# jarek1992/raytracer_project

Hardware: AMD Instinct MI355X
Metric: Msamples/sec (rays·bounces) (higher is better)
Workload: dtype f64

## Files before the change

raytracer_project_amd/csrc/zr_build.h:

```cpp
#pragma once
#include <hip/hip_runtime_api.h>
#include <stdint.h>

#include <vector>

#include "zr_device_types.h"

namespace zr {

struct BuildSceneIn {
    const double* spheres = nullptr; const uint32_t* sphere_mat = nullptr;
    const double* tri_v = nullptr; const double* tri_n = nullptr; const uint32_t* tri_mat = nullptr;
    const double* cubes = nullptr; const uint32_t* cube_mat = nullptr;
    const zr_medium* media = nullptr; const zr_xform_op* ops = nullptr;
    const double* group_box = nullptr;
};

struct BuildParams {
    float ct = 1.0f;
    float ck[8] = {1, 1.5f, 1, 3, 3, 1.5f, 16, 1};
    int max_leaf = 4;
    int leaf_cap[8] = {0, 0, 1, 1, 1, 1, 1, 0};
    float open_ratio = 1.25f;
    int radius = 16;
    int top_clusters = 16384;
};

struct BuildPrimOut {
    double* spheres = nullptr; uint32_t* sphere_mat = nullptr;
    double* tri_v = nullptr; double* tri_s = nullptr;
    double* cubes = nullptr; uint32_t* cube_mat = nullptr;
    double* pcubes = nullptr; uint32_t* pcube_mat = nullptr;
    DInstance* insts = nullptr; uint32_t* inst_group = nullptr;
    uint32_t base[8] = {0, 0, 0, 0, 0, 0, 0, 0};
    uint32_t* src[8] = {};
};

struct BuiltTree {
    NodePair* pairs = nullptr; uint32_t n_pairs = 0;
    NodeQ* quads = nullptr; uint32_t n_quads = 0;
    NodeF root{};
    double box[6] = {0, 0, 0, 0, 0, 0};
    uint32_t depth = 0;
    uint32_t quad_depth = 0;
    uint32_t demand = 0;
    bool quant_ok = true;
    uint32_t cnt[8] = {0, 0, 0, 0, 0, 0, 0, 0};
    std::vector<uint32_t> compound;
    double ms[8] = {0, 0, 0, 0, 0, 0, 0, 0};
    uint32_t ploc_iterations = 0;
    bool want_boxes = false;
    std::vector<float> dbg_boxes;
};

class DeviceBuilder {
public:
    explicit DeviceBuilder(hipStream_t stream) : st_(stream) {}
    ~DeviceBuilder();
    DeviceBuilder(const DeviceBuilder&) = delete;
    DeviceBuilder& operator=(const DeviceBuilder&) = delete;
    static size_t scratch_bytes(uint32_t n);
    hipError_t reserve(size_t bytes);
    hipError_t build(const BuildSceneIn& in, const zr_object* d_objects, const uint8_t* d_code, uint32_t first_triangle, uint32_t n,
                     const BuildParams& prm, bool root_in_array, const BuildPrimOut& out, const uint32_t* d_run_demand,
                     uint32_t depth_limit, bool stats, BuiltTree& t);
    hipError_t relocate(const BuiltTree& t, NodePair* pairs_dst, uint32_t pair_off, NodeQ* quads_dst, uint32_t quad_off);
    hipError_t patch_instances(DInstance* insts, const uint32_t* inst_group, uint32_t n, const uint32_t* d_run_root, const uint32_t* d_run_qroot);
    const char* error() const { return err_; }
    bool wants_host() const { return use_host_; }
    void* alloc_keep(size_t bytes);
private:
    hipStream_t st_;
    unsigned char* arena_ = nullptr; size_t arena_bytes_ = 0;
// ... 7 lines not shown
```

raytracer_project_amd/csrc/zr_build.hip:

```cpp
#include <cstring>
#include <hip/hip_runtime.h>
#include <rocprim/device/device_radix_sort.hpp>
#include <rocprim/device/device_scan.hpp>
#include <rocprim/iterator/counting_iterator.hpp>
#include <rocprim/iterator/transform_iterator.hpp>

#include <algorithm>
#include <chrono>
#include <cstdio>
#include <vector>

#include "zr_build.h"
#include "zr_bvh.h"

namespace zr {
namespace {

constexpr uint32_t NONE = 0xFFFFFFFFu;
constexpr int MAX_R = 32;
constexpr uint32_t M_KIND = 7u, M_UNIFORM = 8u, M_LEAF = 16u;

struct PBox { float lo[3]; uint32_t kind; float hi[3]; uint32_t pad; };
struct Cl { float lo[3]; uint32_t node; float hi[3]; uint32_t pad; };
struct BNode { float lo[3]; uint32_t left; float hi[3]; uint32_t right; };
static_assert(sizeof(PBox) == 32 && sizeof(Cl) == 32 && sizeof(BNode) == 32, "32-byte records: two 16-byte accesses");

struct Params {
    float ct; float ck[8]; int max_leaf; int cap[8]; float open_ratio; int radius;
};

__device__ __forceinline__ float f_down(double x) { return nextafterf(__double2float_rd(x), -__builtin_huge_valf()); }
__device__ __forceinline__ float f_up(double x) { return nextafterf(__double2float_ru(x), __builtin_huge_valf()); }
__device__ __forceinline__ float half_area(const float* lo, const float* hi) {
    const float dx = hi[0] - lo[0], dy = hi[1] - lo[1], dz = hi[2] - lo[2];
    return dx * dy + dy * dz + dz * dx;
}

struct DBox { double lo[3], hi[3]; };

__device__ DBox prim_box(const BuildSceneIn& in, uint32_t type, uint32_t idx);
__device__ DBox apply_op_box(const zr_xform_op& op, const DBox& b) {
    DBox o;
    if (op.kind == ZR_OP_TRANSLATE) { for (int k = 0; k < 3; k++) { o.lo[k] = b.lo[k] + op.a[k]; o.hi[k] = b.hi[k] + op.a[k]; } return o; }
    if (op.kind == ZR_OP_SCALE) {
        for (int k = 0; k < 3; k++) { const double a0 = b.lo[k] * op.a[k], a1 = b.hi[k] * op.a[k]; o.lo[k] = fmin(a0, a1); o.hi[k] = fmax(a0, a1); }
        return o;
    }
    if (op.kind == ZR_OP_MATERIAL) return b;
    const double sn = op.a[0], co = op.a[1];
    const int ia = op.kind == ZR_OP_ROTATE_X ? 1 : 0, ib = op.kind == ZR_OP_ROTATE_Z ? 1 : 2, ic = 3 - ia - ib;
    const double a0 = ia == 0 ? b.lo[0] : b.lo[1], a1 = ia == 0 ? b.hi[0] : b.hi[1];
// ... 367 lines not shown
        for (int k = 0; k < nk; k++) { lo[k] = bn[kids[k]].lo[ax]; hi[k] = bn[kids[k]].hi[ax]; }
        if (!quant_axis(lo, hi, nk, nq.origin[ax], nq.scale[ax], ql[ax], qh[ax])) return false;
        for (int k = 0; k < nk; k++) { nq.q[ax] |= ql[ax][k] << (8 * k); nq.q[3 + ax] |= qh[ax][k] << (8 * k); }
    }
    worst = 1;
    for (int k = 0; k < nk; k++) {
        double d[3];
        for (int ax = 0; ax < 3; ax++) d[ax] = plane_val(nq.origin[ax], nq.scale[ax], (int)qh[ax][k]) - plane_val(nq.origin[ax], nq.scale[ax], (int)ql[ax][k]);
        const double aq = d[0] * d[1] + d[1] * d[2] + d[2] * d[0];
        const BNode b = bn[kids[k]];
        const double at = (double)half_area(b.lo, b.hi);
        const float rr = at > 0 ? (float)(aq / at) : (aq > 0 ? 3.0e38f : 1.0f);
        if (!(rr <= worst)) worst = rr;
    }
    return true;
}

struct PlanOut {
    uint32_t counter;
    uint32_t quant_fail;
    uint32_t quad_depth;
    uint32_t kept_closed;
    uint32_t root_demand;
    uint32_t pad_[3];
    NodeF root;
};

__device__ __forceinline__ uint32_t leaf_ref(const uint32_t* __restrict__ nmeta, const uint32_t* __restrict__ ncount, const uint32_t* __restrict__ leaf_pos, uint32_t node) {
    return ZR_REF_LEAF | ((nmeta[node] & M_KIND) << 28) | ((ncount[node] - 1u) << 24) | leaf_pos[node];
}

__global__ __launch_bounds__(256) void k_plan(const BNode* __restrict__ bn, const uint32_t* __restrict__ nmeta, const uint32_t* __restrict__ ncount,
                                              const uint32_t* __restrict__ leaf_pos, uint32_t node_lo, uint32_t node_hi, uint32_t root, int root_in_array, float open_ratio,
                                              const zr_object* __restrict__ objs, const uint32_t* __restrict__ run_demand,
                                              uint32_t* __restrict__ qroot, uint32_t* __restrict__ qlevel, uint32_t* __restrict__ qinst, NodeQ* __restrict__ quads,
                                              PlanOut* __restrict__ po) {
    const uint32_t id = node_lo + blockIdx.x * 256 + threadIdx.x;
    if (id >= node_hi) return;
    const bool is_root = id == root;
    const bool fp32_root = is_root && !root_in_array;
    const uint32_t me = qroot[id];
    if (!fp32_root && me == NONE) return;
    uint32_t kids[4]; int nk = 0;
    NodeQ nq;
    for (int ax = 0; ax < 3; ax++) { nq.origin[ax] = 0; nq.scale[ax] = 1; }
    for (int k = 0; k < 6; k++) nq.q[k] = 0;
    float worst = 1;
    if (nmeta[id] & M_LEAF) {
        kids[nk++] = id;
        if (!fp32_root && !quantise(bn, kids, nk, nq, worst)) atomicExch(&po->quant_fail, 1u);
    } else {
        const BNode b = bn[id];
        kids[0] = b.left; kids[1] = b.right; nk = 2;
        if (!fp32_root && !quantise(bn, kids, nk, nq, worst)) atomicExch(&po->quant_fail, 1u);
        while (nk < 4) {
            int best = -1; float ba = -1;
            for (int k = 0; k < nk; k++) {
                if (nmeta[kids[k]] & M_LEAF) continue;
                const BNode c = bn[kids[k]];
                const float ar = half_area(c.lo, c.hi);
                if (ar > ba) { ba = ar; best = k; }
            }
            if (best < 0) break;
            uint32_t trial[4];
            for (int k = 0; k < nk; k++) trial[k] = kids[k];
            const BNode ob = bn[kids[best]];
            trial[best] = ob.left; trial[nk] = ob.right;
            if (!fp32_root) {
                NodeQ tq = nq; float w = 1;
                if (!quantise(bn, trial, nk + 1, tq, w)) { atomicExch(&po->quant_fail, 1u); break; }
                if (w > open_ratio && w > worst) { atomicAdd(&po->kept_closed, 1u); break; }
                nq = tq; worst = w;
            }
            for (int k = 0; k <= nk; k++) kids[k] = trial[k];
            nk++;
        }
    }
    int n_inner = 0;
    for (int k = 0; k < nk; k++) if (!(nmeta[kids[k]] & M_LEAF)) n_inner++;
    uint32_t next = n_inner ? atomicAdd(&po->counter, (uint32_t)n_inner) : 0u;
    const uint32_t my_level = fp32_root ? 0u : qlevel[me];
    uint32_t refs[4] = {ZR_REF_EMPTY, ZR_REF_EMPTY, ZR_REF_EMPTY, ZR_REF_EMPTY};
    uint32_t inst_demand = 0;
    for (int k = 0; k < nk; k++) {
        const uint32_t c = kids[k];
        if (nmeta[c] & M_LEAF) {
            refs[k] = leaf_ref(nmeta, ncount, leaf_pos, c);
            if ((nmeta[c] & M_KIND) == ZR_KIND_INSTANCE && run_demand && objs) {
                uint32_t q = c;
                while (bn[q].right != NONE) q = bn[q].left;
                const uint32_t g = objs[bn[q].left].index;
                const uint32_t d = 1u + run_demand[g];
                if (d > inst_demand) inst_demand = d;
            }
        } else { refs[k] = next; qroot[c] = next; qlevel[next] = my_level + 1u; next++; }
    }
    if (n_inner) atomicMax(&po->quad_depth, my_level + 1u);
    if (fp32_root) {
        NodeF rf;
// ... 212 lines not shown
}
__global__ __launch_bounds__(256) void k_fill_u32(uint32_t* __restrict__ a, size_t n, uint32_t v) {
    const size_t i = (size_t)blockIdx.x * 256 + threadIdx.x;
    if (i < n) a[i] = v;
}

inline dim3 grid_for(size_t n) { return dim3((unsigned)((n + 255) / 256)); }
double now_s() { return std::chrono::duration<double>(std::chrono::steady_clock::now().time_since_epoch()).count(); }

}

DeviceBuilder::~DeviceBuilder() {
    if (arena_) (void)hipFree(arena_);
    for (void* p : keep_) (void)hipFree(p);
}
void* DeviceBuilder::alloc_keep(size_t bytes) {
    void* p = nullptr;
    if (hipMalloc(&p, bytes < 64 ? 64 : bytes) != hipSuccess) { (void)hipGetLastError(); return nullptr; }
    keep_.push_back(p);
    return p;
}
size_t DeviceBuilder::scratch_bytes(uint32_t n) {
    const size_t N = 2 * (size_t)n + 2;
    return (size_t)n * (32 + 16 + 8 + 64 + 4 + 1 + 4 + 1 + 4 + 4 + 4 + 4 + 4 + 4 + 8) + N * (32 + 4 + 4 + 4 + 4 + 4 + 4) + (size_t)n * 24 + (64u << 20);
}
hipError_t DeviceBuilder::reserve(size_t bytes) {
    if (bytes <= arena_bytes_) return hipSuccess;
    if (arena_) { (void)hipStreamSynchronize(st_); (void)hipFree(arena_); arena_ = nullptr; arena_bytes_ = 0; }
    hipError_t e = hipMalloc((void**)&arena_, bytes);
    if (e != hipSuccess) { (void)hipGetLastError(); err_ = "out of device memory for the build's scratch"; return e; }
    arena_bytes_ = bytes;
    return hipSuccess;
}

hipError_t DeviceBuilder::build(const BuildSceneIn& in, const zr_object* d_objects, const uint8_t* d_code, uint32_t first_triangle, uint32_t n,
                                const BuildParams& bp, bool root_in_array, const BuildPrimOut& out, const uint32_t* d_run_demand, uint32_t depth_limit,
                                bool stats, BuiltTree& t) {
    hipError_t e;
    err_ = ""; use_host_ = false;
    if (n == 0) { err_ = "empty tree"; use_host_ = true; return hipErrorInvalidValue; }
    Params prm;
    prm.ct = bp.ct; prm.max_leaf = bp.max_leaf < 1 ? 1 : (bp.max_leaf > 16 ? 16 : bp.max_leaf); prm.open_ratio = bp.open_ratio;
    prm.radius = bp.radius < 1 ? 1 : (bp.radius > MAX_R ? MAX_R : bp.radius);
    for (int k = 0; k < 8; k++) { prm.ck[k] = bp.ck[k]; prm.cap[k] = bp.leaf_cap[k]; }
    const size_t N = 2 * (size_t)n;
    const uint32_t nb_max = (n + 255) / 256;
    PBox* pbox; uint64_t *keys_a, *keys_b; uint32_t *vals_a, *vals_b; Cl *cl_a, *cl_b; BNode* bn;
    uint32_t *parent, *ncount, *nmeta, *leaf_pos, *qroot, *nn, *blk_keep, *blk_new, *keep_off, *new_off, *dfs_obj, *rank, *scanned, *qlevel, *qinst, *qdem, *compound, *state;
    float* ncost; uint8_t *act, *dfs_kind; PlanOut* po; void* tmp; size_t tmp_bytes = 0;
    uint32_t *qinst_plan, *qmap, *qscan; NodeQ* quads_plan;
    auto layout = [&](unsigned char* base) -> size_t {
        unsigned char* at = base;
        auto take = [&](size_t bytes) { void* p = at; at += (bytes + 255) / 256 * 256; return p; };
        pbox = (PBox*)take((size_t)n * sizeof(PBox));
        keys_a = (uint64_t*)take((size_t)n * 8); keys_b = (uint64_t*)take((size_t)n * 8);
        vals_a = (uint32_t*)take((size_t)n * 4); vals_b = (uint32_t*)take((size_t)n * 4);
        cl_a = (Cl*)take((size_t)n * sizeof(Cl)); cl_b = (Cl*)take((size_t)n * sizeof(Cl));
        bn = (BNode*)take(N * sizeof(BNode));
        parent = (uint32_t*)take(N * 4); ncount = (uint32_t*)take(N * 4); nmeta = (uint32_t*)take(N * 4);
        ncost = (float*)take(N * 4);
        leaf_pos = (uint32_t*)take(N * 4); qroot = (uint32_t*)take(N * 4);
        nn = (uint32_t*)take((size_t)n * 4); act = (uint8_t*)take(n);
        blk_keep = (uint32_t*)take((size_t)nb_max * 4); blk_new = (uint32_t*)take((size_t)nb_max * 4);
        keep_off = (uint32_t*)take((size_t)nb_max * 4); new_off = (uint32_t*)take((size_t)nb_max * 4);
        dfs_obj = (uint32_t*)take((size_t)n * 4); dfs_kind = (uint8_t*)take(n);
        rank = (uint32_t*)take((size_t)n * 4); scanned = (uint32_t*)take((size_t)n * 4);
        qlevel = (uint32_t*)take((size_t)n * 4); qinst = (uint32_t*)take((size_t)n * 4); qdem = (uint32_t*)take((size_t)n * 4);
        qinst_plan = (uint32_t*)take((size_t)n * 4); qmap = (uint32_t*)take((size_t)n * 4); qscan = (uint32_t*)take(N * 4);
        quads_plan = (NodeQ*)take((size_t)n * sizeof(NodeQ));
        compound = (uint32_t*)take((size_t)n * 8);
        state = (uint32_t*)take(256);
        po = (PlanOut*)take(sizeof(PlanOut));
        if (tmp_bytes == 0) {
            size_t a = 0, b = 0, c = 0;
            (void)rocprim::radix_sort_pairs(nullptr, a, keys_a, keys_b, vals_a, vals_b, (size_t)n, 0, 63, st_);
            (void)rocprim::exclusive_scan(nullptr, b, rocprim::make_transform_iterator(dfs_kind, IsKind{0}), scanned, 0u, (size_t)n, rocprim::plus<uint32_t>(), st_);
            (void)rocprim::exclusive_scan(nullptr, c, rocprim::make_transform_iterator(rocprim::make_counting_iterator<uint32_t>(0u), InnerFlag{nmeta, 0}), scanned, 0u,
                                          (size_t)n, rocprim::plus<uint32_t>(), st_);
            size_t d = 0;
            (void)rocprim::exclusive_scan(nullptr, d, rocprim::make_transform_iterator(rocprim::make_counting_iterator<uint32_t>(0u), QRootFlag{qroot, 0}), qscan, 0u, N,
                                          rocprim::plus<uint32_t>(), st_);
            if (d > c) c = d;
            tmp_bytes = (a > b ? (a > c ? a : c) : (b > c ? b : c)) + 4096;
        }
        tmp = take(tmp_bytes);
        return (size_t)(at - base);
    };
    const size_t need = layout(nullptr);
    if ((e = reserve(need)) != hipSuccess) return e;
    (void)layout(arena_);
    double t0 = now_s();
    auto lap = [&](int k) { if (stats) { (void)hipStreamSynchronize(st_); const double t1 = now_s(); t.ms[k] += (t1 - t0) * 1e3; t0 = t1; } };
// ... 118 lines not shown
    const uint32_t quad_cap = n;
    NodeQ* quads = (NodeQ*)alloc_keep((size_t)quad_cap * sizeof(NodeQ));
    NodePair* pairs = (NodePair*)alloc_keep((size_t)n * sizeof(NodePair));
    if (!quads || !pairs) { err_ = "out of device memory for the tree's records"; return hipErrorOutOfMemory; }
    hipLaunchKernelGGL(k_fill_u32, grid_for(N), dim3(256), 0, st_, qroot, N, NONE);
    PlanOut h_po_in; std::memset(&h_po_in, 0, sizeof h_po_in);
    h_po_in.counter = root_in_array ? 1u : 0u;
    if ((e = hipMemcpyAsync(po, &h_po_in, sizeof h_po_in, hipMemcpyHostToDevice, st_)) != hipSuccess) return e;
    if ((e = hipMemsetAsync(qinst_plan, 0, (size_t)n * 4, st_)) != hipSuccess) return e;
    if ((e = hipMemsetAsync(qinst, 0, (size_t)n * 4, st_)) != hipSuccess) return e;
    if ((e = hipMemsetAsync(qdem, 0, (size_t)n * 4, st_)) != hipSuccess) return e;
    auto renumber = [&]() -> hipError_t {
        auto flags = rocprim::make_transform_iterator(rocprim::make_counting_iterator<uint32_t>(0u), QRootFlag{qroot, root});
        hipError_t er = rocprim::exclusive_scan(tmp, tmp_bytes, flags, qscan, 0u, (size_t)n_nodes, rocprim::plus<uint32_t>(), st_);
        if (er != hipSuccess) { err_ = "scan failed"; return er; }
        hipLaunchKernelGGL(k_qmap, grid_for(n_nodes), dim3(256), 0, st_, qroot, qscan, n_nodes, qmap);
        hipLaunchKernelGGL(k_qpermute, grid_for(quad_cap), dim3(256), 0, st_, quads_plan, quads, qinst_plan, qinst, qmap, quad_cap, po);
        return hipSuccess;
    };
    if (root_in_array) {
        if ((e = hipMemsetAsync(qroot + root, 0, 4, st_)) != hipSuccess) return e;
        if ((e = hipMemsetAsync(qlevel, 0, 4, st_)) != hipSuccess) return e;
    }
    if (n == 1) {
        hipLaunchKernelGGL(k_plan, dim3(1), dim3(256), 0, st_, bn, nmeta, ncount, leaf_pos, root, root + 1, root, root_in_array ? 1 : 0, prm.open_ratio, d_objects, d_run_demand,
                           qroot, qlevel, qinst_plan, quads_plan, po);
        if ((e = renumber()) != hipSuccess) return e;
        hipLaunchKernelGGL(k_demand, dim3(1), dim3(256), 0, st_, qroot, root, root + 1, root, root_in_array ? 1 : 0, quads, qinst, qdem, po);
    } else {
        for (size_t b = batch_start.size() - 1; b-- > 0;) {
            const uint32_t lo = batch_start[b], hi = batch_start[b + 1];
            hipLaunchKernelGGL(k_plan, grid_for(hi - lo), dim3(256), 0, st_, bn, nmeta, ncount, leaf_pos, lo, hi, root, root_in_array ? 1 : 0, prm.open_ratio, d_objects,
                               d_run_demand, qroot, qlevel, qinst_plan, quads_plan, po);
        }
        if ((e = renumber()) != hipSuccess) return e;
        for (size_t b = 0; b + 1 < batch_start.size(); b++) {
            const uint32_t lo = batch_start[b], hi = batch_start[b + 1];
            hipLaunchKernelGGL(k_demand, grid_for(hi - lo), dim3(256), 0, st_, qroot, lo, hi, root, root_in_array ? 1 : 0, quads, qinst, qdem, po);
        }
    }
    lap(4);
    uint32_t n_pairs = 1;
    if (n >= 2) {
        uint32_t h_root_meta = 0;
        if ((e = hipMemcpyAsync(&h_root_meta, nmeta + root, 4, hipMemcpyDeviceToHost, st_)) != hipSuccess) return e;
        if ((e = hipStreamSynchronize(st_)) != hipSuccess) return e;
        if (h_root_meta & M_LEAF) hipLaunchKernelGGL(k_pair_leaf_root, dim3(1), dim3(1), 0, st_, bn, nmeta, ncount, leaf_pos, root, pairs);
        else {
            auto flags = rocprim::make_transform_iterator(rocprim::make_counting_iterator<uint32_t>(0u), InnerFlag{nmeta, root});
            uint32_t* prank = scanned;
            if ((e = rocprim::exclusive_scan(tmp, tmp_bytes, flags, prank, 0u, (size_t)(n - 1), rocprim::plus<uint32_t>(), st_)) != hipSuccess) { err_ = "scan failed"; return e; }
            hipLaunchKernelGGL(k_pairs, grid_for(n - 1), dim3(256), 0, st_, bn, nmeta, ncount, leaf_pos, prank, n, pairs);
            uint32_t last = 0, last_meta = 0;
            if ((e = hipMemcpyAsync(&last, prank + (n - 2), 4, hipMemcpyDeviceToHost, st_)) != hipSuccess) return e;
            if ((e = hipMemcpyAsync(&last_meta, nmeta + n, 4, hipMemcpyDeviceToHost, st_)) != hipSuccess) return e;
            if ((e = hipStreamSynchronize(st_)) != hipSuccess) return e;
            n_pairs = last + ((last_meta & M_LEAF) ? 0u : 1u);
        }
    } else hipLaunchKernelGGL(k_pair_leaf_root, dim3(1), dim3(1), 0, st_, bn, nmeta, ncount, leaf_pos, root, pairs);
    lap(5);
    if ((e = hipMemsetAsync(state + 20, 0, 4, st_)) != hipSuccess) return e;
    hipLaunchKernelGGL(k_emit, grid_for(n), dim3(256), 0, st_, in, d_objects, d_code, first_triangle, n, dfs_obj, dfs_kind, rank, out, compound, state + 20);
    uint32_t n_compound = 0;
    BNode h_root;
    PlanOut h_po;
    if ((e = hipMemcpyAsync(&h_po, po, sizeof h_po, hipMemcpyDeviceToHost, st_)) != hipSuccess) return e;
    if ((e = hipMemcpyAsync(&n_compound, state + 20, 4, hipMemcpyDeviceToHost, st_)) != hipSuccess) return e;
    if ((e = hipMemcpyAsync(&h_root, bn + root, sizeof h_root, hipMemcpyDeviceToHost, st_)) != hipSuccess) return e;
    if ((e = hipStreamSynchronize(st_)) != hipSuccess) return e;
    t.compound.resize((size_t)n_compound * 2);
    if (n_compound && (e = hipMemcpy(t.compound.data(), compound, (size_t)n_compound * 8, hipMemcpyDeviceToHost)) != hipSuccess) return e;
    lap(6);
    t.pairs = pairs; t.n_pairs = n_pairs; t.quads = quads; t.n_quads = h_po.counter;
    t.root = h_po.root; t.quad_depth = h_po.quad_depth; t.demand = h_po.root_demand; t.quant_ok = h_po.quant_fail == 0;
    for (int k = 0; k < 3; k++) { t.box[k] = h_root.lo[k]; t.box[3 + k] = h_root.hi[k]; }
    if ((e = hipGetLastError()) != hipSuccess) { err_ = "a build kernel failed to launch"; return e; }
    return hipSuccess;
}

hipError_t DeviceBuilder::relocate(const BuiltTree& t, NodePair* pairs_dst, uint32_t pair_off, NodeQ* quads_dst, uint32_t quad_off) {
    if (t.n_pairs) hipLaunchKernelGGL(k_reloc_pairs, grid_for(t.n_pairs), dim3(256), 0, st_, t.pairs, t.n_pairs, pair_off, pairs_dst);
    if (t.n_quads) hipLaunchKernelGGL(k_reloc_quads, grid_for(t.n_quads), dim3(256), 0, st_, t.quads, t.n_quads, quad_off, quads_dst);
    return hipGetLastError();
}
hipError_t DeviceBuilder::patch_instances(DInstance* insts, const uint32_t* inst_group, uint32_t n, const uint32_t* d_run_root, const uint32_t* d_run_qroot) {
    if (n) hipLaunchKernelGGL(k_patch_insts, grid_for(n), dim3(256), 0, st_, insts, inst_group, n, d_run_root, d_run_qroot);
    return hipGetLastError();
}

}
```

raytracer_project_amd/csrc/zr_commit.cpp:

```cpp
#include "zr_flatten.h"

namespace {

int finish_commit(zr_scene* s, const CommitSummary& cs, size_t n_objs) {
    int rc;
    if (std::getenv("ZR_QUANT_STATS")) std::fprintf(stderr, "[zr] 4-wide nodes: %zu quantised (64 B) + FP32 root; %zu children kept closed for the grid\n", cs.n_quads, cs.kept_closed);
    s->quad_ok = cs.quant_ok && cs.n_quads < (1u << 31) && cs.max_leaf <= 16 && cs.n_sph < (1u << 24) && cs.n_tri < (1u << 24) && cs.n_cube < (1u << 24) &&
                 cs.n_media < (1u << 24) && cs.n_wrapped < (1u << 24) && cs.n_pcube < (1u << 24) && cs.n_insts < (1u << 24);
    if ((rc = s->d_ops.upload(s->ops.data(), s->ops.size()))) return rc;
    {
        std::vector<zr_material> mats = s->materials;
        auto tex_uses_uv = [&](uint32_t id) {
            std::vector<uint32_t> todo{id}; int guard = 0;
            while (!todo.empty() && guard++ < 4096) {
                uint32_t t = todo.back(); todo.pop_back();
                if (t >= s->textures.size()) continue;
                const zr_texture& tx = s->textures[t];
                if (tx.kind >= ZR_TEX_IMAGE_U8) return true;
                if (tx.kind == ZR_TEX_CHECKER) { todo.push_back(tx.odd); todo.push_back(tx.even); }
            }
            return guard >= 4096;
        };
        for (zr_material& m : mats) m.pad_ = (m.bump_tex != ZR_NO_TEXTURE || (m.kind != ZR_MAT_DIELECTRIC && tex_uses_uv(m.tex))) ? 1u : 0u;
        if ((rc = s->d_mats.upload(mats))) return rc;
    }
// ... 39 lines not shown
            std::memcpy(&fo.rec[fo.n][7], &idb, 8); std::memcpy(&fo.rec[fo.n][8], &tb, 8);
            fo.n++;
        }
        bool scaled = false;
        for (uint32_t i = 0; i < fo.n; i++) if (fo.kind[i] == ZR_KIND_PCUBE && fo.rec[i][15] != 0.0) scaled = true;
        s->fused = fo; s->fused_ok = !scaled;
    }
    {
        if (cs.n_insts) s->leaf_level = 3;
        else if (cs.n_wrapped || !cs.plain_media) s->leaf_level = 2;
        else if (cs.n_cube || cs.n_pcube || cs.n_media) s->leaf_level = 1;
        else s->leaf_level = 0;
        const int force = (int)env_double("ZR_EXTEND_LEVEL", -1);
        if (force > s->leaf_level && force <= 3) s->leaf_level = force;
        bool lean = s->leaf_level == 0 && env_double("ZR_SHADE_LEAN", 1) != 0;
        for (const zr_material& m : s->materials) {
            if (m.kind != ZR_MAT_LAMBERTIAN && m.kind != ZR_MAT_METAL && m.kind != ZR_MAT_DIELECTRIC && m.kind != ZR_MAT_LIGHT) lean = false;
            if (m.bump_tex != ZR_NO_TEXTURE) lean = false;
            if (m.kind != ZR_MAT_DIELECTRIC && (m.tex >= s->textures.size() || s->textures[m.tex].kind != ZR_TEX_SOLID)) lean = false;
        }
        d.shade_lean = lean ? 1u : 0u;
    }
    s->stack_demand = cs.stack_demand;
    if (std::getenv("ZR_QUANT_STATS")) std::fprintf(stderr, "[zr] 4-wide tree: depth %d, worst-case traversal stack %u entries\n", cs.quad_depth, s->stack_demand);
    s->stats[0] = cs.n_pairs; s->stats[1] = (uint64_t)cs.max_depth; s->stats[2] = n_objs;
    s->stats[3] = cs.n_pairs * sizeof(zr::NodePair) + cs.n_quads * sizeof(zr::NodeQ) + (cs.n_sph * 4 + cs.n_tri * (ZR_TRI_STRIDE + 20) + cs.n_cube * 6 + cs.n_pcube * ZR_PCUBE_STRIDE) * 8 +
                  (cs.n_sph + cs.n_cube) * 4 + s->texels.size();
    s->builder = cs.builder;
    if (std::getenv("ZR_COMMIT_HASH")) {
        (void)hipDeviceSynchronize();
        auto fnv = [](const void* dev, size_t bytes) -> unsigned long long {
            std::vector<unsigned char> h(bytes);
            unsigned long long x = 1469598103934665603ull;
            if (bytes && hipMemcpy(h.data(), dev, bytes, hipMemcpyDeviceToHost) == hipSuccess) for (unsigned char b : h) { x ^= b; x *= 1099511628211ull; }
            return x;
        };
        std::fprintf(stderr, "[zr] commit hash (%s): quads %016llx (%zu), pairs %016llx (%zu)\n", cs.builder, fnv(s->d_quads.p, cs.n_quads * sizeof(zr::NodeQ)), cs.n_quads,
                     fnv(s->d_nodes.p, cs.n_pairs * sizeof(zr::NodePair)), cs.n_pairs);
    }
    s->committed = true;
    if (s->borrowed) {
        s->spheres.drop(); s->sphere_mat.drop(); s->tri_v.drop(); s->tri_n.drop(); s->tri_mat.drop(); s->cubes.drop(); s->cube_mat.drop();
        s->media.drop(); s->ops.drop(); s->objects.drop(); s->texels.drop(); s->objects_set = false; s->borrowed = false; s->released = true;
    }
    return ZR_OK;
}

// ... 66 lines not shown
        (rc = send(r_objs, objs.data(), objs.size())) || (rc = send(r_tri_mat, s->tri_mat.data(), s->tri_mat.size())) ||
        (rc = send(r_sph, s->spheres.data(), s->spheres.size())) || (rc = send(r_sph_mat, s->sphere_mat.data(), s->sphere_mat.size())) ||
        (rc = send(r_cubes, s->cubes.data(), s->cubes.size())) || (rc = send(r_cube_mat, s->cube_mat.data(), s->cube_mat.size())) ||
        (rc = send(r_media, s->media.data(), s->media.size())) || (rc = s->d_ops.upload(s->ops.data(), s->ops.size())) || (rc = send(r_code, code.data(), code.size()))) return rc;
    if ((rc = s->d_spheres.alloc(n_sph * 4)) || (rc = s->d_sphere_mat.alloc(n_sph)) || (rc = s->d_tri_v.alloc(n_tri * ZR_TRI_STRIDE)) || (rc = s->d_tri_s.alloc(n_tri * 20)) ||
        (rc = s->d_cubes.alloc(n_cube * 6)) || (rc = s->d_cube_mat.alloc(n_cube)) || (rc = s->d_pcubes.alloc(n_pcube * ZR_PCUBE_STRIDE)) || (rc = s->d_pcube_mat.alloc(n_pcube)) ||
        (rc = s->d_insts.alloc(n_insts)) || (rc = d_inst_group.alloc(n_insts))) return rc;
    phase("upload as given");
    zr::BuildSceneIn in;
    in.spheres = r_sph.p; in.sphere_mat = r_sph_mat.p; in.tri_v = r_tri_v.p; in.tri_n = r_tri_n.p; in.tri_mat = r_tri_mat.p;
    in.cubes = r_cubes.p; in.cube_mat = r_cube_mat.p; in.media = r_media.p; in.ops = s->d_ops.p;
    zr::BuildParams bp;
    bp.ct = (float)env_double("ZR_BVH_COST_TRAVERSE", 1.0);
    const double ck[8] = {env_double("ZR_BVH_COST_SPHERE", 1.0), env_double("ZR_BVH_COST_TRI", 1.5), env_double("ZR_BVH_COST_CUBE", 1.0),
                          env_double("ZR_BVH_COST_MEDIUM", 3.0), env_double("ZR_BVH_COST_WRAPPED", 3.0), env_double("ZR_BVH_COST_PCUBE", 1.5),
                          env_double("ZR_BVH_COST_GROUP", 16.0), 1};
    for (int k = 0; k < 8; k++) bp.ck[k] = (float)ck[k];
    bp.max_leaf = (int)env_double("ZR_BVH_MAX_LEAF", 4);
    const int big = (int)env_double("ZR_BVH_MAX_LEAF_BIG", 1);
    const int leaf_cap[8] = {0, 0, big, big, big, big, 1, 0};
    for (int k = 0; k < 8; k++) bp.leaf_cap[k] = leaf_cap[k];
    bp.open_ratio = (float)env_double("ZR_BVH_OPEN_RATIO", 1.25);
    bp.radius = (int)env_double("ZR_BVH_PLOC_RADIUS", 16);
    {
        const double top_env = env_double("ZR_BVH_TOP", -1);
        bp.top_clusters = top_env >= 0 ? (int)top_env : (int)std::min<size_t>(65536, std::max<size_t>(4096, (size_t)n / 64));
    }
    DevBuf<uint32_t> d_src[8];
    {
        const size_t sz[8] = {n_sph, n_tri, n_cube, n_media, n_wrapped, n_pcube, n_insts, 0};
        for (int k = 0; k < 7; k++) {
            if ((rc = d_src[k].alloc(sz[k]))) return rc;
            HIP_OK(hipMemsetAsync(d_src[k].p, 0xFF, std::max<size_t>(sz[k], 1) * 4, st));
        }
    }
    zr::BuildPrimOut out;
    for (int k = 0; k < 7; k++) out.src[k] = d_src[k].p;
    out.spheres = s->d_spheres.p; out.sphere_mat = s->d_sphere_mat.p; out.tri_v = s->d_tri_v.p; out.tri_s = s->d_tri_s.p;
    out.cubes = s->d_cubes.p; out.cube_mat = s->d_cube_mat.p; out.pcubes = s->d_pcubes.p; out.pcube_mat = s->d_pcube_mat.p;
    out.insts = s->d_insts.p; out.inst_group = d_inst_group.p;
    auto builder = std::make_shared<zr::DeviceBuilder>(st);
    auto build_fail = [&](hipError_t e) {
        if (builder->wants_host()) { std::fprintf(stderr, "[zr] device BVH build: %s\n", builder->error()); return (int)ZR_FALLBACK_HOST; }
        if (e == hipErrorOutOfMemory) {
            (void)hipGetLastError();
            std::fprintf(stderr, "[zr] device BVH build: out of device memory (%s): host builder\n", builder->error());
// ... 8 lines not shown
    std::vector<uint32_t> run_demand(ng), run_tri_base(ng);
    {
        size_t at = cnt[ZR_PRIM_TRIANGLE];
        for (size_t g = 0; g < ng; g++) {
            const zr_group& grp = s->groups[g];
            run_tri_base[g] = (uint32_t)at; at += grp.triangle_count;
            zr::BuildPrimOut go = out;
            go.base[ZR_PRIM_TRIANGLE] = run_tri_base[g];
            hipError_t e = builder->build(in, nullptr, nullptr, grp.first_triangle, grp.triangle_count, bp, true, go, nullptr, ZR_STACK_DEPTH - 2, false, runs[g]);
            if (e != hipSuccess) return build_fail(e);
            for (int k = 0; k < 6; k++) gbox[g * 6 + k] = runs[g].box[k];
            run_demand[g] = runs[g].demand;
        }
    }
    if (ng) { if ((rc = r_gbox.upload(gbox)) || (rc = d_run_demand.upload(run_demand))) return rc; in.group_box = r_gbox.p; }
    phase("groups' trees");
    zr::BuiltTree world;
    world.want_boxes = std::getenv("ZR_BUILD_CHECK") != nullptr;
    {
        hipError_t e = builder->build(in, r_objs.p, r_code.p, 0, n, bp, false, out, ng ? d_run_demand.p : nullptr, ZR_STACK_DEPTH - 2, commit_stats, world);
        if (e != hipSuccess) return build_fail(e);
    }
    if (commit_stats)
        std::fprintf(stderr, "[zr] device build: boxes+keys %.2f, sort %.2f, PLOC %.2f (%u iterations), order %.2f, 4-wide %.2f, pairs %.2f, emit %.2f ms; depth %u, %u pairs, %u quads\n",
                     world.ms[0], world.ms[1], world.ms[2], world.ploc_iterations, world.ms[3], world.ms[4], world.ms[5], world.ms[6], world.depth, world.n_pairs, world.n_quads);
    if (world.want_boxes) {
        std::vector<zr::BuildBox> gb(ng);
        for (size_t g = 0; g < ng; g++) for (int k = 0; k < 3; k++) { gb[g].lo[k] = gbox[g * 6 + k]; gb[g].hi[k] = gbox[g * 6 + 3 + k]; }
        Boxer boxer{*s, &gb};
        size_t bad = 0;
        for (uint32_t k = 0; k < n; k++) {
            const zr::BuildBox hb = boxer.chain(objs[k].type, objs[k].index, objs[k].chain_first, objs[k].chain_count);
            const float* d = &world.dbg_boxes[(size_t)k * 8];
            bool ok = true;
            for (int a = 0; a < 3; a++) if (!((double)d[a] <= hb.lo[a]) || !((double)d[4 + a] >= hb.hi[a])) ok = false;
            if (!ok && bad++ < 8)
                std::fprintf(stderr, "[zr] BUILD_CHECK: object %u (type %u, chain %u): device box [%g %g %g | %g %g %g] does not contain the host's [%g %g %g | %g %g %g]\n", k, objs[k].type,
                             objs[k].chain_count, d[0], d[1], d[2], d[4], d[5], d[6], hb.lo[0], hb.lo[1], hb.lo[2], hb.hi[0], hb.hi[1], hb.hi[2]);
        }
        if (bad) return fail(ZR_E_DEVICE, "ZR_BUILD_CHECK: %zu of %u object boxes computed on the device do not contain the host's", bad, n);
    }
    for (int k = 0; k < 8; k++)
        if (world.cnt[k] != cnt[k]) return fail(ZR_E_DEVICE, "device BVH build: %u leaf primitives of kind %d, expected %u (internal error)", world.cnt[k], k, cnt[k]);
    phase("world tree");
    size_t n_pairs = world.n_pairs, n_quads = world.n_quads;
    std::vector<uint32_t> run_root(ng), run_qroot(ng);
    for (size_t g = 0; g < ng; g++) { run_root[g] = (uint32_t)n_pairs; run_qroot[g] = (uint32_t)n_quads; n_pairs += runs[g].n_pairs; n_quads += runs[g].n_quads; }
    if ((rc = s->d_nodes.alloc(n_pairs)) || (rc = s->d_quads.alloc(n_quads))) return rc;
// ... 37 lines not shown
            }
        }
        if (fl.n_sph != n_sph || fl.n_tri != n_tri || fl.n_cube != n_cube || fl.n_media != n_media)
            return fail(ZR_E_DEVICE, "device BVH build: compound objects do not add up (internal error)");
        for (size_t k = 0; k < n_media; k++) if (fl.media[k].chain_count != 0) plain_media = false;
        auto up = [&](void* dst, const void* src, size_t bytes) -> int { if (bytes) HIP_OK(hipMemcpyAsync(dst, src, bytes, hipMemcpyHostToDevice, st)); return ZR_OK; };
        if ((rc = up(s->d_spheres.p + b_sph * 4, &fl.spheres[b_sph * 4], (n_sph - b_sph) * 32)) || (rc = up(s->d_sphere_mat.p + b_sph, &fl.sphere_mat[b_sph], (n_sph - b_sph) * 4)) ||
            (rc = up(s->d_tri_v.p + b_tri * ZR_TRI_STRIDE, &fl.tri_v[b_tri * ZR_TRI_STRIDE], (n_tri - b_tri) * ZR_TRI_STRIDE * 8)) ||
            (rc = up(s->d_tri_s.p + b_tri * 20, &fl.tri_s[b_tri * 20], (n_tri - b_tri) * 160)) ||
            (rc = up(s->d_cubes.p + b_cube * 6, &fl.cubes[b_cube * 6], (n_cube - b_cube) * 48)) || (rc = up(s->d_cube_mat.p + b_cube, &fl.cube_mat[b_cube], (n_cube - b_cube) * 4)) ||
            (rc = up(s->d_media.p, fl.media.data(), n_media * sizeof(zr::DMedium))) || (rc = up(s->d_wrapped.p, fl.wrapped.data(), n_wrapped * sizeof(zr::DWrapped)))) return rc;
        HIP_OK(hipStreamSynchronize(st));
    }
    HIP_OK(hipStreamSynchronize(st));
    for (int k = 0; k < 8; k++) {
        s->leaf_src[k].assign(d_src[k].n, 0xFFFFFFFFu);
        if (d_src[k].n) HIP_OK(hipMemcpy(s->leaf_src[k].data(), d_src[k].p, d_src[k].n * 4, hipMemcpyDeviceToHost));
    }
    phase("node arrays + compound");
    cs.root = world.root; cs.quant_ok = world.quant_ok;
    for (const zr::BuiltTree& r : runs) cs.quant_ok = cs.quant_ok && r.quant_ok;
    cs.n_pairs = n_pairs; cs.n_quads = n_quads; cs.n_sph = n_sph; cs.n_tri = n_tri; cs.n_cube = n_cube; cs.n_pcube = n_pcube;
    cs.n_media = n_media; cs.n_wrapped = n_wrapped; cs.n_insts = n_insts; cs.plain_media = plain_media;
    cs.stack_demand = world.demand; cs.quad_depth = (int)world.quad_depth; cs.max_depth = (int)world.depth; cs.max_leaf = bp.max_leaf;
    for (int k = 0; k < 8; k++) cs.leaf_cnt[k] = cnt[k];
    cs.builder = "device (PLOC)";
    {
        struct Trash { std::shared_ptr<zr::DeviceBuilder> b; DevBuf<double> a0, a1, a2, a3, a4; DevBuf<uint32_t> u0, u1, u2, u3, u4, u5, u6; DevBuf<zr_medium> m; DevBuf<zr_object> o; DevBuf<uint8_t> c; int device; };
        auto t = std::make_shared<Trash>();
        t->device = s->ctx->device;
        t->b = std::move(builder);
        std::swap(t->a0, r_sph); std::swap(t->a1, r_tri_v); std::swap(t->a2, r_tri_n); std::swap(t->a3, r_cubes); std::swap(t->a4, r_gbox);
        std::swap(t->u0, r_sph_mat); std::swap(t->u1, r_tri_mat); std::swap(t->u2, r_cube_mat); std::swap(t->u3, d_inst_group); std::swap(t->u4, d_run_demand);
        std::swap(t->u5, d_run_root); std::swap(t->u6, d_run_qroot); std::swap(t->m, r_media); std::swap(t->o, r_objs); std::swap(t->c, r_code);
        s->ctx->free_later([t]() mutable { (void)hipSetDevice(t->device); t.reset(); });
    }
    phase("release");
    return ZR_OK;
}

}

extern "C" {

zr_scene* zr_scene_create(zr_ctx* c) {
    if (!c) { fail(ZR_E_INVALID, "null context"); return nullptr; }
// ... 352 lines not shown
```

Baseline: 6229.

## Collapse binary BVH to 4-wide tree with SAH-optimal dynamic programming

Result: no change. 6278 (median of 6 runs) (+0.8%).

```diff
diff --git a/raytracer_project_amd/csrc/zr_build.h b/raytracer_project_amd/csrc/zr_build.h
--- a/raytracer_project_amd/csrc/zr_build.h
+++ b/raytracer_project_amd/csrc/zr_build.h
@@ -23,6 +23,8 @@
     int leaf_cap[8] = {0, 0, 1, 1, 1, 1, 1, 0};
     float open_ratio = 1.25f;
     int radius = 16;
+    float cq = 1.0f;
+    bool collapse_opt = true;
     int top_clusters = 16384;
 };
 
@@ -49,6 +51,8 @@
     std::vector<uint32_t> compound;
     double ms[8] = {0, 0, 0, 0, 0, 0, 0, 0};
     uint32_t ploc_iterations = 0;
+    uint32_t kept_closed = 0;
+    uint32_t dp_fallback = 0;
     bool want_boxes = false;
     std::vector<float> dbg_boxes;
 };
diff --git a/raytracer_project_amd/csrc/zr_build.hip b/raytracer_project_amd/csrc/zr_build.hip
--- a/raytracer_project_amd/csrc/zr_build.hip
+++ b/raytracer_project_amd/csrc/zr_build.hip
@@ -12,6 +12,7 @@
 
 #include "zr_build.h"
 #include "zr_bvh.h"
+#include "zr_collapse.h"
 
 namespace zr {
 namespace {
@@ -27,6 +28,7 @@
 
 struct Params {
     float ct; float ck[8]; int max_leaf; int cap[8]; float open_ratio; int radius;
+    float cq; int collapse_opt;
 };
 
 __device__ __forceinline__ float f_down(double x) { return nextafterf(__double2float_rd(x), -__builtin_huge_valf()); }
@@ -440,7 +442,8 @@
     uint32_t quad_depth;
     uint32_t kept_closed;
     uint32_t root_demand;
-    uint32_t pad_[3];
+    uint32_t dp_fallback;
+    uint32_t pad_[2];
     NodeF root;
 };
 
@@ -448,9 +451,19 @@
     return ZR_REF_LEAF | ((nmeta[node] & M_KIND) << 28) | ((ncount[node] - 1u) << 24) | leaf_pos[node];
 }
 
+__global__ __launch_bounds__(256) void k_collapse_dp(const BNode* __restrict__ bn, const uint32_t* __restrict__ nmeta, const uint32_t* __restrict__ ncount,
+                                                     uint32_t node_lo, uint32_t node_hi, Params prm, CollapseDP* __restrict__ dp) {
+    const uint32_t id = node_lo + blockIdx.x * 256 + threadIdx.x;
+    if (id >= node_hi) return;
+    const BNode b = bn[id];
+    const float ar = half_area(b.lo, b.hi);
+    const uint32_t m = nmeta[id];
+    dp[id] = (m & M_LEAF) ? collapse_leaf(ar, prm.ck[m & M_KIND], ncount[id]) : collapse_inner(ar, prm.cq, dp[b.left], dp[b.right]);
+}
+
 __global__ __launch_bounds__(256) void k_plan(const BNode* __restrict__ bn, const uint32_t* __restrict__ nmeta, const uint32_t* __restrict__ ncount,
                                               const uint32_t* __restrict__ leaf_pos, uint32_t node_lo, uint32_t node_hi, uint32_t root, int root_in_array, float open_ratio,
-                                              const zr_object* __restrict__ objs, const uint32_t* __restrict__ run_demand,
+                                              const CollapseDP* __restrict__ dp, const zr_object* __restrict__ objs, const uint32_t* __restrict__ run_demand,
                                               uint32_t* __restrict__ qroot, uint32_t* __restrict__ qlevel, uint32_t* __restrict__ qinst, NodeQ* __restrict__ quads,
                                               PlanOut* __restrict__ po) {
     const uint32_t id = node_lo + blockIdx.x * 256 + threadIdx.x;
@@ -468,31 +481,21 @@
         kids[nk++] = id;
         if (!fp32_root && !quantise(bn, kids, nk, nq, worst)) atomicExch(&po->quant_fail, 1u);
     } else {
-        const BNode b = bn[id];
-        kids[0] = b.left; kids[1] = b.right; nk = 2;
-        if (!fp32_root && !quantise(bn, kids, nk, nq, worst)) atomicExch(&po->quant_fail, 1u);
-        while (nk < 4) {
-            int best = -1; float ba = -1;
-            for (int k = 0; k < nk; k++) {
-                if (nmeta[kids[k]] & M_LEAF) continue;
-                const BNode c = bn[kids[k]];
-                const float ar = half_area(c.lo, c.hi);
-                if (ar > ba) { ba = ar; best = k; }
-            }
-            if (best < 0) break;
-            uint32_t trial[4];
-            for (int k = 0; k < nk; k++) trial[k] = kids[k];
-            const BNode ob = bn[kids[best]];
-            trial[best] = ob.left; trial[nk] = ob.right;
-            if (!fp32_root) {
-                NodeQ tq = nq; float w = 1;
-                if (!quantise(bn, trial, nk + 1, tq, w)) { atomicExch(&po->quant_fail, 1u); break; }
-                if (w > open_ratio && w > worst) { atomicAdd(&po->kept_closed, 1u); break; }
-                nq = tq; worst = w;
-            }
-            for (int k = 0; k <= nk; k++) kids[k] = trial[k];
-            nk++;
-        }
+        auto inner = [&](uint32_t n, uint32_t& l, uint32_t& r) {
+            if (nmeta[n] & M_LEAF) return false;
+            const BNode c = bn[n];
+            l = c.left; r = c.right;
+            return true;
+        };
+        auto area = [&](uint32_t n) { const BNode c = bn[n]; return half_area(c.lo, c.hi); };
+        auto quant = [&](const uint32_t* ids, int m, float& w) { NodeQ tq; return quantise(bn, ids, m, tq, w); };
+        const QuadPlan pl = plan_quad(id, dp, open_ratio, !fp32_root, inner, area, quant);
+        if (pl.quant_fail) atomicExch(&po->quant_fail, 1u);
+        if (pl.kept_closed) atomicAdd(&po->kept_closed, pl.kept_closed);
+        if (pl.fell_back) atomicAdd(&po->dp_fallback, 1u);
+        nk = pl.nk;
+        for (int k = 0; k < nk; k++) kids[k] = pl.kid[k];
+        if (!fp32_root) (void)quantise(bn, kids, nk, nq, worst);
     }
     int n_inner = 0;
     for (int k = 0; k < nk; k++) if (!(nmeta[kids[k]] & M_LEAF)) n_inner++;
@@ -751,7 +754,7 @@
 }
 size_t DeviceBuilder::scratch_bytes(uint32_t n) {
     const size_t N = 2 * (size_t)n + 2;
-    return (size_t)n * (32 + 16 + 8 + 64 + 4 + 1 + 4 + 1 + 4 + 4 + 4 + 4 + 4 + 4 + 8) + N * (32 + 4 + 4 + 4 + 4 + 4 + 4) + (size_t)n * 24 + (64u << 20);
+    return (size_t)n * (32 + 16 + 8 + 64 + 4 + 1 + 4 + 1 + 4 + 4 + 4 + 4 + 4 + 4 + 8) + N * (32 + 4 + 4 + 4 + 4 + 4 + 4 + sizeof(CollapseDP)) + (size_t)n * 24 + (64u << 20);
 }
 hipError_t DeviceBuilder::reserve(size_t bytes) {
     if (bytes <= arena_bytes_) return hipSuccess;
@@ -772,12 +775,13 @@
     prm.ct = bp.ct; prm.max_leaf = bp.max_leaf < 1 ? 1 : (bp.max_leaf > 16 ? 16 : bp.max_leaf); prm.open_ratio = bp.open_ratio;
     prm.radius = bp.radius < 1 ? 1 : (bp.radius > MAX_R ? MAX_R : bp.radius);
     for (int k = 0; k < 8; k++) { prm.ck[k] = bp.ck[k]; prm.cap[k] = bp.leaf_cap[k]; }
+    prm.cq = bp.cq; prm.collapse_opt = bp.collapse_opt ? 1 : 0;
     const size_t N = 2 * (size_t)n;
     const uint32_t nb_max = (n + 255) / 256;
     PBox* pbox; uint64_t *keys_a, *keys_b; uint32_t *vals_a, *vals_b; Cl *cl_a, *cl_b; BNode* bn;
     uint32_t *parent, *ncount, *nmeta, *leaf_pos, *qroot, *nn, *blk_keep, *blk_new, *keep_off, *new_off, *dfs_obj, *rank, *scanned, *qlevel, *qinst, *qdem, *compound, *state;
     float* ncost; uint8_t *act, *dfs_kind; PlanOut* po; void* tmp; size_t tmp_bytes = 0;
-    uint32_t *qinst_plan, *qmap, *qscan; NodeQ* quads_plan;
+    uint32_t *qinst_plan, *qmap, *qscan; NodeQ* quads_plan; CollapseDP* dp;
     auto layout = [&](unsigned char* base) -> size_t {
         unsigned char* at = base;
         auto take = [&](size_t bytes) { void* p = at; at += (bytes + 255) / 256 * 256; return p; };
@@ -797,6 +801,7 @@
         qlevel = (uint32_t*)take((size_t)n * 4); qinst = (uint32_t*)take((size_t)n * 4); qdem = (uint32_t*)take((size_t)n * 4);
         qinst_plan = (uint32_t*)take((size_t)n * 4); qmap = (uint32_t*)take((size_t)n * 4); qscan = (uint32_t*)take(N * 4);
         quads_plan = (NodeQ*)take((size_t)n * sizeof(NodeQ));
+        dp = (CollapseDP*)take(N * sizeof(CollapseDP));
         compound = (uint32_t*)take((size_t)n * 8);
         state = (uint32_t*)take(256);
         po = (PlanOut*)take(sizeof(PlanOut));
@@ -961,16 +966,25 @@
         if ((e = hipMemsetAsync(qroot + root, 0, 4, st_)) != hipSuccess) return e;
         if ((e = hipMemsetAsync(qlevel, 0, 4, st_)) != hipSuccess) return e;
     }
+    const CollapseDP* plan_dp = nullptr;
+    if (prm.collapse_opt && n >= 2) {
+        hipLaunchKernelGGL(k_collapse_dp, grid_for(n), dim3(256), 0, st_, bn, nmeta, ncount, 0u, n, prm, dp);
+        for (size_t b = 0; b + 1 < batch_start.size(); b++) {
+            const uint32_t lo = batch_start[b], hi = batch_start[b + 1];
+            hipLaunchKernelGGL(k_collapse_dp, grid_for(hi - lo), dim3(256), 0, st_, bn, nmeta, ncount, lo, hi, prm, dp);
+        }
+        plan_dp = dp;
+    }
     if (n == 1) {
-        hipLaunchKernelGGL(k_plan, dim3(1), dim3(256), 0, st_, bn, nmeta, ncount, leaf_pos, root, root + 1, root, root_in_array ? 1 : 0, prm.open_ratio, d_objects, d_run_demand,
-                           qroot, qlevel, qinst_plan, quads_plan, po);
+        hipLaunchKernelGGL(k_plan, dim3(1), dim3(256), 0, st_, bn, nmeta, ncount, leaf_pos, root, root + 1, root, root_in_array ? 1 : 0, prm.open_ratio, plan_dp, d_objects,
+                           d_run_demand, qroot, qlevel, qinst_plan, quads_plan, po);
         if ((e = renumber()) != hipSuccess) return e;
         hipLaunchKernelGGL(k_demand, dim3(1), dim3(256), 0, st_, qroot, root, root + 1, root, root_in_array ? 1 : 0, quads, qinst, qdem, po);
     } else {
         for (size_t b = batch_start.size() - 1; b-- > 0;) {
             const uint32_t lo = batch_start[b], hi = batch_start[b + 1];
-            hipLaunchKernelGGL(k_plan, grid_for(hi - lo), dim3(256), 0, st_, bn, nmeta, ncount, leaf_pos, lo, hi, root, root_in_array ? 1 : 0, prm.open_ratio, d_objects,
-                               d_run_demand, qroot, qlevel, qinst_plan, quads_plan, po);
+            hipLaunchKernelGGL(k_plan, grid_for(hi - lo), dim3(256), 0, st_, bn, nmeta, ncount, leaf_pos, lo, hi, root, root_in_array ? 1 : 0, prm.open_ratio, plan_dp,
+                               d_objects, d_run_demand, qroot, qlevel, qinst_plan, quads_plan, po);
         }
         if ((e = renumber()) != hipSuccess) return e;
         for (size_t b = 0; b + 1 < batch_start.size(); b++) {
@@ -1012,6 +1026,7 @@
     lap(6);
     t.pairs = pairs; t.n_pairs = n_pairs; t.quads = quads; t.n_quads = h_po.counter;
     t.root = h_po.root; t.quad_depth = h_po.quad_depth; t.demand = h_po.root_demand; t.quant_ok = h_po.quant_fail == 0;
+    t.kept_closed = h_po.kept_closed; t.dp_fallback = h_po.dp_fallback;
     for (int k = 0; k < 3; k++) { t.box[k] = h_root.lo[k]; t.box[3 + k] = h_root.hi[k]; }
     if ((e = hipGetLastError()) != hipSuccess) { err_ = "a build kernel failed to launch"; return e; }
     return hipSuccess;
diff --git a/raytracer_project_amd/csrc/zr_collapse.h b/raytracer_project_amd/csrc/zr_collapse.h
--- /dev/null
+++ b/raytracer_project_amd/csrc/zr_collapse.h
@@ -0,0 +1,117 @@
+#pragma once
+#include <stdint.h>
+
+#if defined(__HIPCC__) || defined(__CUDACC__)
+#define ZR_HD __host__ __device__
+#else
+#define ZR_HD
+#endif
+
+namespace zr {
+
+struct CollapseDP {
+    float d[4];
+    uint32_t pick;
+};
+
+ZR_HD inline CollapseDP collapse_leaf(float area, float c_prim, uint32_t count) {
+    const float c = area * c_prim * (float)count;
+    CollapseDP o;
+    for (int k = 0; k < 4; k++) o.d[k] = c;
+    o.pick = 0;
+    return o;
+}
+
+ZR_HD inline CollapseDP collapse_inner(float area, float c_node, const CollapseDP& l, const CollapseDP& r) {
+    float s[5] = {0, 0, 0, 0, 0};
+    uint32_t si[5] = {0, 0, 0, 0, 0};
+    for (int k = 2; k <= 4; k++) {
+        s[k] = l.d[0] + r.d[k - 2];
+        si[k] = 1;
+        for (int i = 2; i < k; i++) {
+            const float v = l.d[i - 1] + r.d[k - i - 1];
+            if (v < s[k]) { s[k] = v; si[k] = (uint32_t)i; }
+        }
+    }
+    CollapseDP o;
+    const float c = area * c_node + s[4];
+    o.d[0] = c;
+    o.pick = si[4] << 6;
+    for (int k = 2; k <= 4; k++) {
+        if (s[k] < c) { o.d[k - 1] = s[k]; o.pick |= si[k] << (2 * (k - 2)); }
+        else o.d[k - 1] = c;
+    }
+    return o;
+}
+
+ZR_HD inline uint32_t collapse_pick(const CollapseDP& p, int k) { return k == 0 ? (p.pick >> 6) & 3u : (p.pick >> (2 * (k - 2))) & 3u; }
+
+struct QuadPlan {
+    uint32_t kid[4];
+    int nk = 0;
+    float worst = 1;
+    bool quant_fail = false;
+    bool fell_back = false;
+    uint32_t kept_closed = 0;
+};
+
+template <class Inner, class Area, class Quant>
+ZR_HD inline QuadPlan plan_quad(uint32_t node, const CollapseDP* dp, float open_ratio, bool guard, Inner inner, Area area, Quant quant) {
+    QuadPlan p;
+    uint32_t l = 0, r = 0;
+    (void)inner(node, l, r);
+    p.kid[0] = l; p.kid[1] = r; p.nk = 2;
+    float base = 1;
+    bool base_ok = true;
+    if (guard) { base_ok = quant(p.kid, 2, base); if (!base_ok) p.quant_fail = true; }
+    if (dp) {
+        uint32_t sn[4], sk[4]; int sp = 0;
+        uint32_t kid[4]; int nk = 0;
+        const uint32_t i0 = collapse_pick(dp[node], 0);
+        sn[sp] = r; sk[sp] = 4 - i0; sp++;
+        sn[sp] = l; sk[sp] = i0; sp++;
+        while (sp > 0) {
+            sp--;
+            const uint32_t n = sn[sp], k = sk[sp];
+            uint32_t a, b;
+            const uint32_t i = k >= 2 ? collapse_pick(dp[n], (int)k) : 0u;
+            if (i == 0 || !inner(n, a, b)) { kid[nk++] = n; continue; }
+            sn[sp] = b; sk[sp] = k - i; sp++;
+            sn[sp] = a; sk[sp] = i; sp++;
+        }
+        float w = 1;
+        if (!guard || (base_ok && quant(kid, nk, w) && (w <= open_ratio || w <= base))) {
+            for (int k = 0; k < nk; k++) p.kid[k] = kid[k];
+            p.nk = nk; p.worst = w;
+            return p;
+        }
+        p.fell_back = true;
+    }
+    float worst = base;
+    while (p.nk < 4) {
+        int best = -1; float ba = -1;
+        uint32_t ol = 0, orr = 0;
+        for (int k = 0; k < p.nk; k++) {
+            uint32_t a, b;
+            if (!inner(p.kid[k], a, b)) continue;
+            const float ar = area(p.kid[k]);
+            if (ar > ba) { ba = ar; best = k; ol = a; orr = b; }
+        }
+        if (best < 0) break;
+        uint32_t trial[4];
+        for (int k = 0; k < p.nk; k++) trial[k] = p.kid[k];
+        trial[best] = ol; trial[p.nk] = orr;
+        if (guard) {
+            float w = 1;
+            if (!quant(trial, p.nk + 1, w)) { p.quant_fail = true; break; }
+            if (w > open_ratio && w > worst) { p.kept_closed++; break; }
+            worst = w;
+        }
+        for (int k = 0; k <= p.nk; k++) p.kid[k] = trial[k];
+        p.nk++;
+    }
+    p.worst = worst;
+    return p;
+}
+
+}
diff --git a/raytracer_project_amd/csrc/zr_commit.cpp b/raytracer_project_amd/csrc/zr_commit.cpp
--- a/raytracer_project_amd/csrc/zr_commit.cpp
+++ b/raytracer_project_amd/csrc/zr_commit.cpp
@@ -1,6 +1,58 @@
 #include "zr_flatten.h"
 
 namespace {
+
+void report_tree_quality(const CommitSummary& cs, const zr::NodeQ* d_quads) {
+    std::vector<zr::NodeQ> q(cs.n_quads);
+    (void)hipDeviceSynchronize();
+    if (cs.n_quads && hipMemcpy(q.data(), d_quads, cs.n_quads * sizeof(zr::NodeQ), hipMemcpyDeviceToHost) != hipSuccess) { (void)hipGetLastError(); return; }
+    auto harea = [](const double* lo, const double* hi) { const double dx = hi[0] - lo[0], dy = hi[1] - lo[1], dz = hi[2] - lo[2]; return dx * dy + dy * dz + dz * dx; };
+    const zr::NodeF& r = cs.root;
+    double root_lo[3] = {kInf, kInf, kInf}, root_hi[3] = {-kInf, -kInf, -kInf};
+    bool any_inner = false;
+    for (int c = 0; c < 4; c++) any_inner = any_inner || (r.ref[c] != ZR_REF_EMPTY && !(r.ref[c] & ZR_REF_LEAF));
+    for (int c = 0; c < 4; c++) {
+        if (r.ref[c] == ZR_REF_EMPTY || (any_inner && (r.ref[c] & ZR_REF_LEAF))) continue;
+        const double lo[3] = {r.lox[c], r.loy[c], r.loz[c]}, hi[3] = {r.hix[c], r.hiy[c], r.hiz[c]};
+        for (int a = 0; a < 3; a++) { root_lo[a] = std::min(root_lo[a], lo[a]); root_hi[a] = std::max(root_hi[a], hi[a]); }
+    }
+    const double a_root = harea(root_lo, root_hi);
+    if (!(a_root > 0)) return;
+    double e_nodes = 1, e_prims = 0;
+    size_t nodes = 1, children = 0, hist[17] = {};
+    std::vector<std::pair<uint32_t, double>> todo;
+    auto child = [&](uint32_t ref, double area, bool priced) {
+        if (ref == ZR_REF_EMPTY) return;
+        children++;
+        if (ref & ZR_REF_LEAF) { const uint32_t cnt = ((ref >> 24) & 15u) + 1u; hist[cnt]++; if (priced) e_prims += cnt * area / a_root; }
+        else if (ref < q.size()) todo.emplace_back(ref, area);
+    };
+    for (int c = 0; c < 4; c++) {
+        const double lo[3] = {r.lox[c], r.loy[c], r.loz[c]}, hi[3] = {r.hix[c], r.hiy[c], r.hiz[c]};
+        child(r.ref[c], harea(lo, hi), !any_inner);
+    }
+    while (!todo.empty()) {
+        const auto [qi, area] = todo.back(); todo.pop_back();
+        const zr::NodeQ& nq = q[qi];
+        nodes++; e_nodes += area / a_root;
+        for (int c = 0; c < 4; c++) {
+            double lo[3], hi[3];
+            for (int a = 0; a < 3; a++) {
+                lo[a] = (double)nq.origin[a] + (double)((nq.q[a] >> (8 * c)) & 0xFFu) * (double)nq.scale[a];
+                hi[a] = (double)nq.origin[a] + (double)((nq.q[3 + a] >> (8 * c)) & 0xFFu) * (double)nq.scale[a];
+            }
+            child(nq.ref[c], harea(lo, hi), true);
+        }
+    }
+    size_t in_leaves = 0, leaf_objects = 0;
+    for (int k = 1; k <= 16; k++) in_leaves += (size_t)k * hist[k];
+    for (int k = 0; k < 8; k++) leaf_objects += cs.leaf_cnt[k];
+    std::fprintf(stderr, "[zr] 4-wide tree quality: SAH cost %.6f = %.6f node visits + %.6f primitive tests per ray; %zu nodes, %.3f children per node; "
+                         "%zu of %zu primitives in leaves; leaves by size:",
+                 e_nodes + e_prims, e_nodes, e_prims, nodes, (double)children / (double)nodes, in_leaves, leaf_objects);
+    for (int k = 1; k <= 16; k++) if (hist[k]) std::fprintf(stderr, " %d:%zu", k, hist[k]);
+    std::fprintf(stderr, "\n");
+}
 
 int finish_commit(zr_scene* s, const CommitSummary& cs, size_t n_objs) {
     int rc;
@@ -86,7 +138,10 @@
         d.shade_lean = lean ? 1u : 0u;
     }
     s->stack_demand = cs.stack_demand;
-    if (std::getenv("ZR_QUANT_STATS")) std::fprintf(stderr, "[zr] 4-wide tree: depth %d, worst-case traversal stack %u entries\n", cs.quad_depth, s->stack_demand);
+    if (std::getenv("ZR_QUANT_STATS")) {
+        std::fprintf(stderr, "[zr] 4-wide tree: depth %d, worst-case traversal stack %u entries\n", cs.quad_depth, s->stack_demand);
+        report_tree_quality(cs, s->d_quads.p);
+    }
     s->stats[0] = cs.n_pairs; s->stats[1] = (uint64_t)cs.max_depth; s->stats[2] = n_objs;
     s->stats[3] = cs.n_pairs * sizeof(zr::NodePair) + cs.n_quads * sizeof(zr::NodeQ) + (cs.n_sph * 4 + cs.n_tri * (ZR_TRI_STRIDE + 20) + cs.n_cube * 6 + cs.n_pcube * ZR_PCUBE_STRIDE) * 8 +
                   (cs.n_sph + cs.n_cube) * 4 + s->texels.size();
@@ -199,6 +254,8 @@
     for (int k = 0; k < 8; k++) bp.leaf_cap[k] = leaf_cap[k];
     bp.open_ratio = (float)env_double("ZR_BVH_OPEN_RATIO", 1.25);
     bp.radius = (int)env_double("ZR_BVH_PLOC_RADIUS", 16);
+    bp.collapse_opt = env_double("ZR_BVH_OPT", 1) != 0;
+    bp.cq = (float)env_double("ZR_BVH_COST_QUAD", 1.0);
     {
         const double top_env = env_double("ZR_BVH_TOP", -1);
         bp.top_clusters = top_env >= 0 ? (int)top_env : (int)std::min<size_t>(65536, std::max<size_t>(4096, (size_t)n / 64));
@@ -253,8 +310,10 @@
         if (e != hipSuccess) return build_fail(e);
     }
     if (commit_stats)
-        std::fprintf(stderr, "[zr] device build: boxes+keys %.2f, sort %.2f, PLOC %.2f (%u iterations), order %.2f, 4-wide %.2f, pairs %.2f, emit %.2f ms; depth %u, %u pairs, %u quads\n",
-                     world.ms[0], world.ms[1], world.ms[2], world.ploc_iterations, world.ms[3], world.ms[4], world.ms[5], world.ms[6], world.depth, world.n_pairs, world.n_quads);
+        std::fprintf(stderr, "[zr] device build: boxes+keys %.2f, sort %.2f, PLOC %.2f (%u iterations), order %.2f, 4-wide %.2f, pairs %.2f, emit %.2f ms; depth %u, %u pairs, %u quads"
+                             " (%s collapse, %u plans refused by the grid)\n",
+                     world.ms[0], world.ms[1], world.ms[2], world.ploc_iterations, world.ms[3], world.ms[4], world.ms[5], world.ms[6], world.depth, world.n_pairs, world.n_quads,
+                     bp.collapse_opt ? "SAH-optimal" : "greedy", world.dp_fallback);
     if (world.want_boxes) {
         std::vector<zr::BuildBox> gb(ng);
         for (size_t g = 0; g < ng; g++) for (int k = 0; k < 3; k++) { gb[g].lo[k] = gbox[g * 6 + k]; gb[g].hi[k] = gbox[g * 6 + 3 + k]; }
@@ -338,6 +397,7 @@
     for (const zr::BuiltTree& r : runs) cs.quant_ok = cs.quant_ok && r.quant_ok;
     cs.n_pairs = n_pairs; cs.n_quads = n_quads; cs.n_sph = n_sph; cs.n_tri = n_tri; cs.n_cube = n_cube; cs.n_pcube = n_pcube;
     cs.n_media = n_media; cs.n_wrapped = n_wrapped; cs.n_insts = n_insts; cs.plain_media = plain_media;
+    cs.kept_closed = world.kept_closed;
     cs.stack_demand = world.demand; cs.quad_depth = (int)world.quad_depth; cs.max_depth = (int)world.depth; cs.max_leaf = bp.max_leaf;
     for (int k = 0; k < 8; k++) cs.leaf_cnt[k] = cnt[k];
     cs.builder = "device (PLOC)";
```
